# psipred/DMPfold2

Measured on AMD Instinct MI355X. Metric: structures/s at L=300, N_seq=2000, 10 iters+100 min, higher is better.
Workload: dtype f32 with full-width operands on the bf16 matrix cores (option precision = 2): convolution operands split exactly into 3 bf16 pieces (24 significand bits), the 6 piece products above 2^-24 accumulated in f32 by v_mfma_f32_32x32x16_bf16; vertical GRU the same way (3 bf16 pieces per operand, 6 products

## Files before the change

dmpfold2_amd/csrc/vgru.h:

```cpp
#pragma once
#include "common.h"

namespace dmp {

typedef float f32x16 __attribute__((ext_vector_type(16)));
typedef _Float16 vg_f16x8 __attribute__((ext_vector_type(8)));

struct VStatic {
  const uint4* wx[2];
  const uint4* wh[2];
  const float* bias[2];
  float inv_scale[2];
  float* hT[2][2];
  uint16_t* hH[2][2];
};
constexpr int VG_TB = 32;


__host__ __device__ inline int vgru_pitch(int L) { return (L + VG_TB - 1) / VG_TB * VG_TB; }

typedef unsigned vg_u32x4 __attribute__((ext_vector_type(4)));

constexpr int VG_MAX_MEMBERS = 8;

struct VMember { const uint8_t* msa; int N, L, tile0, pad; };
struct VGroupRec { int t0, t_end, nmem, pad; VMember mem[VG_MAX_MEMBERS]; };
static_assert(sizeof(VGroupRec) <= 256, "dmp_ctx_create sizes vgru_run for 256 bytes");

typedef float vp_f32x4 __attribute__((ext_vector_type(4)));
constexpr int VP_WL0_SLOTS = 4 * 4 * 6 * 64;
constexpr int VP_RED_SLOTS = 4 * 14 * 64;
constexpr int VP_TAB_FLOATS = 3 * 24 * 16;
constexpr int VP_LDS_BYTES = (VP_WL0_SLOTS + VP_RED_SLOTS) * 16 + VP_TAB_FLOATS * 4;
constexpr int VP_MAX_XCD_TILES = 64;
constexpr int VP_GRID = 256;
struct VPSync { unsigned count[8]; unsigned pad[24]; unsigned flag[8][32]; };
static_assert(sizeof(VPSync) == 128 + 1024, "VPSync layout");
constexpr unsigned VP_BARRIER_SPINS = 800000u;
constexpr unsigned VP_BARRIER_SPINS_FIRST = 8u * VP_BARRIER_SPINS;

__device__ __forceinline__ bool vp_claim_slice(VPSync* __restrict__ sync, int* __restrict__ fault, int barrier, int tid,
                                               int* sh_u, int* sh_abort, unsigned& xcc, int& u) {
  if (barrier) {
    asm volatile("s_getreg_b32 %0, hwreg(HW_REG_XCC_ID)" : "=s"(xcc));
    xcc &= 7u;
    if (tid == 0) {
      *sh_u = (int)__hip_atomic_fetch_add(&sync->count[xcc], 1u, __ATOMIC_RELAXED, __HIP_MEMORY_SCOPE_AGENT);
      *sh_abort = 0;
    }
  } else {
    xcc = blockIdx.x & 7u;
    if (tid == 0) { *sh_u = (int)(blockIdx.x >> 3); *sh_abort = 0; }
  }
  __syncthreads();
  u = *sh_u;
  if (u >= 32) {
    if (tid == 0) atomicOr(fault, DMP_FAULT_VGRU_HANDOFF);
    return false;
  }
  return true;
}

__device__ __forceinline__ bool vp_tile_table(const VGroupRec* __restrict__ rec, int nmem, int c_lo, int c_hi, int tid,
                                              int* __restrict__ fault, int (*sh_tile)[4], unsigned long long* sh_msa) {
  if (c_hi - c_lo > VP_MAX_XCD_TILES) {
    if (tid == 0) atomicOr(fault, DMP_FAULT_VGRU_HANDOFF);
    return false;
  }
  for (int i = tid; i < c_hi - c_lo; i += 256) {
    const int tile = c_lo + i;
    int mi = 0;
    for (int m = 1; m < VG_MAX_MEMBERS; ++m)
      if (m < nmem && tile >= rec->mem[m].tile0) mi = m;
    sh_tile[i][0] = rec->mem[mi].N;
    sh_tile[i][1] = rec->mem[mi].L;
    sh_tile[i][2] = (tile - rec->mem[mi].tile0) * VG_TB;
    sh_tile[i][3] = mi;
  }
  if (tid < VG_MAX_MEMBERS) sh_msa[tid] = tid < nmem ? (unsigned long long)rec->mem[tid].msa : 0ull;
  __syncthreads();
  return true;
}

__device__ __forceinline__ int vp_next_active(const int (*sh_tile)[4], int c_lo, int c_hi, int ct, int t) {
  for (; ct < c_hi; ++ct) {
    const int N = __builtin_amdgcn_readfirstlane(sh_tile[ct - c_lo][0]);
    if (t < N || (t >= 1 && t <= N)) break;
  }
  return ct;
}

__device__ __forceinline__ void vp_store_partials(vp_f32x4* red, int w, int lane, const vp_f32x4 (&a0)[3][2],
                                                  const vp_f32x4 (&a1)[4][2]) {
#pragma unroll
  for (int g = 0; g < 3; ++g)
#pragma unroll
    for (int nt = 0; nt < 2; ++nt) red[(w * 14 + g * 2 + nt) * 64 + lane] = a0[g][nt];
#pragma unroll
  for (int g = 0; g < 4; ++g)
#pragma unroll
    for (int nt = 0; nt < 2; ++nt) red[(w * 14 + 6 + g * 2 + nt) * 64 + lane] = a1[g][nt];
}

__device__ __forceinline__ vp_f32x4 vp_quarter_sum(const vp_f32x4* red, int a, int flane) {
  return ((red[(0 * 14 + a) * 64 + flane] + red[(1 * 14 + a) * 64 + flane]) + red[(2 * 14 + a) * 64 + flane]) +
         red[(3 * 14 + a) * 64 + flane];
}

__device__ __forceinline__ vp_f32x4 vp_onehot_term(const float* tab, int g, int code, int fg) {
  const float* t = tab + (g * 24 + code) * 16 + 4 * fg;
  return vp_f32x4{t[0], t[1], t[2], t[3]};
}

__device__ __forceinline__ float vp_gru_cell(float s_r, float s_z, float s_hn, float s_in, float b_r, float b_z, float b_in,
                                             float b_hn, float h) {
  const float rg = 1.0f / (1.0f + expf(-(s_r + b_r)));
  const float zg = 1.0f / (1.0f + expf(-(s_z + b_z)));
  const float ng = tanhf((s_in + b_in) + rg * (s_hn + b_hn));
  return (h - ng) * zg + ng;
}

__device__ __forceinline__ bool vp_row_barrier(VPSync* __restrict__ sync, int* __restrict__ fault, unsigned xcc, int u, int w,
                                               int lane, int tid, int t, int t_lo, int* sh_abort) {
  asm volatile("s_waitcnt vmcnt(0)" ::: "memory");
  __syncthreads();
  const unsigned epoch = (unsigned)(t - t_lo + 1);
  if (tid == 0) asm volatile("global_store_dword %0, %1, off" :: "v"(&sync->flag[xcc][u]), "v"(epoch) : "memory");
  if (w == 0) {
    const unsigned* fp = &sync->flag[xcc][lane & 31];
    bool ok = false;
    const unsigned bound = t == t_lo ? VP_BARRIER_SPINS_FIRST : VP_BARRIER_SPINS;
    for (unsigned spins = 0; spins < bound && !ok; ++spins) {
      unsigned v;
      asm volatile("global_load_dword %0, %1, off sc1\n\ts_waitcnt vmcnt(0)" : "=v"(v) : "v"(fp) : "memory");
      ok = __builtin_amdgcn_ballot_w64(v < epoch) == 0ull;
    }
    if (!ok && lane == 0) { atomicOr(fault, DMP_FAULT_VGRU_HANDOFF); *sh_abort = 1; }
  }
  __syncthreads();
  return *sh_abort != 0;
}


struct VStaticF32 {
  const float4* wh0;
  const float4* wx1;
  const float4* wh1;
  const float* wx0;
  const float* bias[2];
  float* hT[2][2];
  uint4* wq;
};
typedef void (*vgru_f32_kernel_t)(VStaticF32, const VGroupRec*, VPSync*, int*, int, int, int, int);

inline int vgru_f32_launch(vgru_f32_kernel_t kernel, dmp_ctx* lead, int t_lo, int t_hi, hipStream_t s) {
  const int nt = lead->vg_ntiles;
  if (t_hi > lead->vg_maxN + 1) t_hi = lead->vg_maxN + 1;
  if (t_lo < 0) t_lo = 0;
  if (t_lo >= t_hi) return DMP_OK;
  const Weights& W = lead->W;
  VStaticF32 st{};
  st.wh0 = reinterpret_cast<const float4*>(W.v_f32[0]);
  st.wx1 = reinterpret_cast<const float4*>(W.v_f32[1]);
  st.wh1 = reinterpret_cast<const float4*>(W.v_f32[2]);
  st.wx0 = W.v_wx0f;
  st.bias[0] = W.v_b0; st.bias[1] = W.v_b1;
  for (int l = 0; l < 2; ++l)
    for (int p = 0; p < 2; ++p) st.hT[l][p] = lead->hT[l][p];
  st.wq = reinterpret_cast<uint4*>(lead->vgru_wq);
  const VGroupRec* rec = reinterpret_cast<const VGroupRec*>(lead->vgru_run);
  VPSync* sync = reinterpret_cast<VPSync*>(lead->vgru_sync);
  if (lead->vgru_persist && lead->vgru_persist_ok) {
    CoResident guard(lead, s, true);
    if (guard.status()) return guard.status();
    DMP_HIP(hipMemsetAsync(sync, 0, sizeof(VPSync), s));
    hipLaunchKernelGGL(kernel, dim3(VP_GRID - (lead->vgru_debug_drop_wg ? 1 : 0)), dim3(256), VP_LDS_BYTES, s, st, rec, sync,
                       lead->seq_abort, t_lo, t_hi, nt, 1);
    DMP_LAUNCH_CHECK();
    return guard.done();
  }
  for (int t = t_lo; t < t_hi; ++t)
    hipLaunchKernelGGL(kernel, dim3(VP_GRID), dim3(256), VP_LDS_BYTES, s, st, rec, sync, lead->seq_abort, t, t + 1, nt, 0);
  DMP_LAUNCH_CHECK();
  return DMP_OK;
}

int vgru_f32_group_steps(dmp_ctx* lead, int t_lo, int t_hi, hipStream_t s);
int vgru_f32_kernel_attrs(dmp_ctx* c);
int vgru_x3_group_steps(dmp_ctx* lead, int t_lo, int t_hi, hipStream_t s);
int vgru_x3_kernel_attrs(dmp_ctx* c);

}
```

dmpfold2_amd/csrc/vgru_x3.hip:

```cpp
#include "vgru.h"

namespace dmp {

typedef __bf16 vx_bf16x8 __attribute__((ext_vector_type(8)));

__device__ __forceinline__ void vx_split8(const float (&w)[8], vx_bf16x8 (&p)[3]) {
  float r[8];
#pragma unroll
  for (int e = 0; e < 8; ++e) { const __bf16 h = (__bf16)w[e]; p[0][e] = h; r[e] = w[e] - (float)h; }
#pragma unroll
  for (int e = 0; e < 8; ++e) { const __bf16 h = (__bf16)r[e]; p[1][e] = h; r[e] = r[e] - (float)h; }
#pragma unroll
  for (int e = 0; e < 8; ++e) p[2][e] = (__bf16)r[e];
}

__device__ __forceinline__ vp_f32x4 vx_mfma(vx_bf16x8 a, vx_bf16x8 b, vp_f32x4 c) {
  return __builtin_amdgcn_mfma_f32_16x16x32_bf16(a, b, c, 0, 0, 0);
}

__device__ __forceinline__ float vx_sigmoid(float x) { return 1.0f / (1.0f + expf(-x)); }

constexpr int VX_KS = 4;
constexpr int VX_WQ = 6;
constexpr size_t VX_WQ_BYTES = (size_t)VP_GRID * 4 * VX_KS * VX_WQ * 64 * 16;
static_assert(4 * VX_KS * 3 * 2 * 64 == VP_WL0_SLOTS, "two pieces of layer 0's weights fill the LDS area of the f16 form's pieces");

constexpr int VX_SC1 = 16;

struct VxAddr {
  __amdgpu_buffer_rsrc_t r0, r1, rq;
  unsigned vlane, vq;
  unsigned k4w, krot, Lb;
};

__device__ __forceinline__ void vx_request(vp_f32x4 (&F)[4][2], int u4, unsigned S, unsigned col, const VxAddr& A) {
  const unsigned base = ((A.k4w + 8 * ((S + A.krot) & (VX_KS - 1))) * A.Lb + col + (u4 & 1) * 16) * 16;
#pragma unroll
  for (int h = 0; h < 2; ++h)
    F[u4][h] = __builtin_bit_cast(vp_f32x4, __builtin_amdgcn_raw_buffer_load_b128(u4 < 2 ? A.r1 : A.r0, A.vlane, base + h * A.Lb * 16, VX_SC1));
}

__device__ __forceinline__ void vx_split_octet(const vp_f32x4 (&f)[2], vx_bf16x8 (&q)[3]) {
  const float wv[8] = {f[0][0], f[0][1], f[0][2], f[0][3], f[1][0], f[1][1], f[1][2], f[1][3]};
  vx_split8(wv, q);
}

template <bool ACT0, bool ACT1>
__device__ __forceinline__ void vx_tile_products(vp_f32x4 (&a0)[3][2], vp_f32x4 (&a1)[4][2], const vx_bf16x8 (&PA)[VX_KS][3][3],
                                                 const vx_bf16x8 (&PB)[VX_KS][3][2], vx_bf16x8 (&WB)[3], vx_bf16x8 (&WC)[3],
                                                 const vx_bf16x8* __restrict__ wl0w, vp_f32x4 (&F)[4][2], vx_bf16x8 (&Q)[2][3],
                                                 const VxAddr& A, unsigned tcol, unsigned ncol) {
#pragma unroll
  for (int S = 0; S < VX_KS; ++S) {
    vx_bf16x8 T[3][2];
#pragma unroll
    for (int g = 0; g < 3; ++g) {
      T[g][0] = wl0w[((S * 3 + g) * 2 + 0) * 64];
      T[g][1] = wl0w[((S * 3 + g) * 2 + 1) * 64];
    }
    __builtin_amdgcn_sched_barrier(0);
#pragma unroll
    for (int u4 = 0; u4 < 4; ++u4) {
      const int unit = 4 * S + u4, nt = u4 & 1, cur = unit & 1, nxt = cur ^ 1, n4 = (u4 + 1) & 3;
      vx_bf16x8 (&P)[3] = Q[cur];
      const int nm = u4 < 2 ? (ACT1 ? 18 : 0) : (ACT0 ? 18 : 0) + (ACT1 ? 18 : 0);
#pragma unroll
      for (int pb = 2; pb >= 0; --pb)
#pragma unroll
        for (int pa = 2 - pb; pa >= 0; --pa)
#pragma unroll
          for (int g = 0; g < 3; ++g) {
            if (u4 < 2) {
              if (ACT1) a1[g][nt] = vx_mfma(pa == 2 ? WB[g] : PB[S][g][pa == 2 ? 0 : pa], P[pb], a1[g][nt]);
            } else {
              if (ACT0) a0[g][nt] = vx_mfma(pa == 2 ? WC[g] : T[g][pa == 2 ? 0 : pa], P[pb], a0[g][nt]);
              if (ACT1) a1[g == 2 ? 3 : g][nt] = vx_mfma(PA[S][g][pa], P[pb], a1[g == 2 ? 3 : g][nt]);
            }
          }
      vx_split_octet(F[n4], Q[nxt]);
      vx_request(F, n4, (unit + 5) >> 2 & (VX_KS - 1), unit + 5 < 4 * VX_KS ? tcol : ncol, A);
      if (u4 == 1) {
#pragma unroll
        for (int g = 0; g < 3; ++g)
          WB[g] = __builtin_bit_cast(vx_bf16x8, __builtin_amdgcn_raw_buffer_load_b128(A.rq, A.vq, (((S + 1) & (VX_KS - 1)) * VX_WQ + g) * 1024, 0));
      }
      if (u4 == 3) {
#pragma unroll
        for (int g = 0; g < 3; ++g)
          WC[g] = __builtin_bit_cast(vx_bf16x8, __builtin_amdgcn_raw_buffer_load_b128(A.rq, A.vq, (((S + 1) & (VX_KS - 1)) * VX_WQ + 3 + g) * 1024, 0));
      }
#pragma unroll
      for (int i = 0; i < 36; ++i)
        if (i < nm) {
          __builtin_amdgcn_sched_group_barrier(0x008, 1, 0);
          __builtin_amdgcn_sched_group_barrier(0x002, 3, 0);
        }
      __builtin_amdgcn_sched_barrier(0);
    }
  }
}

__global__ __launch_bounds__(256) __attribute__((amdgpu_waves_per_eu(1, 1)))
void vgru_persist_x3_kernel(VStaticF32 st, const VGroupRec* __restrict__ rec, VPSync* __restrict__ sync,
                            int* __restrict__ fault, int t_lo, int t_hi, int ntiles, int barrier) {
  extern __shared__ __attribute__((aligned(16))) unsigned char vx_smem[];
  vx_bf16x8* wl0 = reinterpret_cast<vx_bf16x8*>(vx_smem);
  vp_f32x4* red = reinterpret_cast<vp_f32x4*>(vx_smem + VP_WL0_SLOTS * 16);
  float* tab = reinterpret_cast<float*>(vx_smem + (VP_WL0_SLOTS + VP_RED_SLOTS) * 16);
  __shared__ int sh_u, sh_abort;
  __shared__ __attribute__((aligned(16))) float sh_bias[2][4][16];
  __shared__ int sh_tile[VP_MAX_XCD_TILES][5];
  __shared__ unsigned long long sh_msa[VG_MAX_MEMBERS];
  const int tid = threadIdx.x, lane = tid & 63;
  const int w = __builtin_amdgcn_readfirstlane(tid >> 6);
  unsigned xcc;
  if (barrier) {
    asm volatile("s_getreg_b32 %0, hwreg(HW_REG_XCC_ID)" : "=s"(xcc));
    xcc &= 7u;
    if (tid == 0) {
      sh_u = (int)__hip_atomic_fetch_add(&sync->count[xcc], 1u, __ATOMIC_RELAXED, __HIP_MEMORY_SCOPE_AGENT);
      sh_abort = 0;
    }
  } else {
    xcc = blockIdx.x & 7u;
    if (tid == 0) { sh_u = (int)(blockIdx.x >> 3); sh_abort = 0; }
  }
  __syncthreads();
  const int u = sh_u;
  if (u >= 32) {
    if (tid == 0) atomicOr(fault, DMP_FAULT_VGRU_HANDOFF);
    return;
  }
  const int j0 = 16 * u, lr = lane & 15, lq = lane >> 4;
  const int Lb = ntiles * VG_TB;
  const int c_lo = (int)(((long long)ntiles * xcc) / 8), c_hi = (int)(((long long)ntiles * (xcc + 1)) / 8);

  vx_bf16x8 PA[VX_KS][3][3], PB[VX_KS][3][2];
  uint4* wqw = st.wq + (size_t)(blockIdx.x * 4 + w) * VX_KS * VX_WQ * 64 + lane;
#pragma unroll
  for (int S = 0; S < VX_KS; ++S)
#pragma unroll
    for (int g = 0; g < 3; ++g) {
      float wa[8], wb[8], wc[8];
#pragma unroll
      for (int h = 0; h < 2; ++h) {
        const int64_t off = (int64_t)(g * 128 + 32 * w + 8 * ((S + u) & (VX_KS - 1)) + 2 * lq + h) * 512 + j0 + lr;
        const float4 a = st.wx1[off], b = st.wh1[off], c = st.wh0[off];
        wa[4 * h + 0] = a.x; wa[4 * h + 1] = a.y; wa[4 * h + 2] = a.z; wa[4 * h + 3] = a.w;
        wb[4 * h + 0] = b.x; wb[4 * h + 1] = b.y; wb[4 * h + 2] = b.z; wb[4 * h + 3] = b.w;
        wc[4 * h + 0] = c.x; wc[4 * h + 1] = c.y; wc[4 * h + 2] = c.z; wc[4 * h + 3] = c.w;
      }
      vx_split8(wa, PA[S][g]);
      vx_bf16x8 pb[3], pc[3];
      vx_split8(wb, pb);
      vx_split8(wc, pc);
      PB[S][g][0] = pb[0];
      PB[S][g][1] = pb[1];
      wl0[(((w * VX_KS + S) * 3 + g) * 2 + 0) * 64 + lane] = pc[0];
      wl0[(((w * VX_KS + S) * 3 + g) * 2 + 1) * 64 + lane] = pc[1];
      wqw[(S * VX_WQ + g) * 64] = __builtin_bit_cast(uint4, pb[2]);
      wqw[(S * VX_WQ + 3 + g) * 64] = __builtin_bit_cast(uint4, pc[2]);
    }
  asm volatile("s_waitcnt vmcnt(0)" ::: "memory");
  const vx_bf16x8* wl0w = wl0 + w * VX_KS * 3 * 2 * 64 + lane;
  if (tid < 128) sh_bias[tid >> 6][(tid >> 4) & 3][tid & 15] = st.bias[tid >> 6][((tid >> 4) & 3) * 512 + j0 + (tid & 15)];
  for (int i = tid; i < 3 * 22 * 16; i += 256) {
    const int g = i / (22 * 16), code = (i / 16) % 22, row = i & 15;
    tab[(g * 24 + code) * 16 + row] = st.wx0[(g * 22 + code) * 512 + j0 + row];
  }
  const int fl = __builtin_amdgcn_readfirstlane(tid >> 7), fg = (tid >> 5) & 3, fc = tid & 31;
  const int flane = 16 * fg + (fc & 15), fnt = fc >> 4;
  const int j4 = j0 + 4 * fg;
  const int nmem = rec->nmem;
  if (c_hi - c_lo > VP_MAX_XCD_TILES) {
    if (tid == 0) atomicOr(fault, DMP_FAULT_VGRU_HANDOFF);
    return;
  }
  for (int i = tid; i < c_hi - c_lo; i += 256) {
    const int tile = c_lo + (i + u) % (c_hi - c_lo);
    int mi = 0;
    for (int m = 1; m < VG_MAX_MEMBERS; ++m)
      if (m < nmem && tile >= rec->mem[m].tile0) mi = m;
    sh_tile[i][0] = rec->mem[mi].N;
    sh_tile[i][1] = rec->mem[mi].L;
    sh_tile[i][2] = (tile - rec->mem[mi].tile0) * VG_TB;
    sh_tile[i][3] = mi;
    sh_tile[i][4] = tile;
  }
  if (tid < VG_MAX_MEMBERS) sh_msa[tid] = tid < nmem ? (unsigned long long)rec->mem[tid].msa : 0ull;
  __syncthreads();
  auto next_active = [&](int ct, int t) {
    for (; ct < c_hi; ++ct) {
      const int N = __builtin_amdgcn_readfirstlane(sh_tile[ct - c_lo][0]);
      if (t < N || (t >= 1 && t <= N)) break;
    }
    return ct;
  };
  const unsigned state_bytes = (unsigned)(128 * Lb * 16);

  VxAddr A;
  A.k4w = (unsigned)(32 * w);
  A.krot = (unsigned)(u & (VX_KS - 1));
  A.Lb = (unsigned)Lb;
  A.vlane = (unsigned)((2 * lq * Lb + lr) * 16);
  A.vq = (unsigned)(lane * 16);
  A.rq = __builtin_amdgcn_make_buffer_rsrc(st.wq + (size_t)(blockIdx.x * 4 + w) * VX_KS * VX_WQ * 64, 0, VX_KS * VX_WQ * 1024, 0x00020000);
  vx_bf16x8 WB[3], WC[3];
#pragma unroll
  for (int g = 0; g < 3; ++g) {
    WB[g] = __builtin_bit_cast(vx_bf16x8, __builtin_amdgcn_raw_buffer_load_b128(A.rq, A.vq, g * 1024, 0));
    WC[g] = __builtin_bit_cast(vx_bf16x8, __builtin_amdgcn_raw_buffer_load_b128(A.rq, A.vq, (3 + g) * 1024, 0));
  }
  for (int t = t_lo; t < t_hi; ++t) {
    const int par = t & 1;
    A.r0 = __builtin_amdgcn_make_buffer_rsrc(st.hT[0][par], 0, state_bytes, 0x00020000);
    A.r1 = __builtin_amdgcn_make_buffer_rsrc(st.hT[1][par ^ 1], 0, state_bytes, 0x00020000);
    const __amdgpu_buffer_rsrc_t rh = fl ? A.r1 : A.r0;
    float* hnext = fl ? st.hT[1][par] : st.hT[0][par ^ 1];
    int ct = next_active(c_lo, t);
    vp_f32x4 F[4][2];
    vx_bf16x8 Q[2][3];
    if (ct < c_hi) {
      const unsigned col0 = (unsigned)(__builtin_amdgcn_readfirstlane(sh_tile[ct - c_lo][4]) * VG_TB);
#pragma unroll
      for (int u4 = 0; u4 < 4; ++u4) vx_request(F, u4, 0, col0, A);
      vx_split_octet(F[0], Q[0]);
      vx_request(F, 0, 1, col0, A);
    }
    while (ct < c_hi) {
      const int nx = next_active(ct + 1, t);
      const int ncol = __builtin_amdgcn_readfirstlane(sh_tile[(nx < c_hi ? nx : ct) - c_lo][4]) * VG_TB;
      const int N = __builtin_amdgcn_readfirstlane(sh_tile[ct - c_lo][0]);
      const int L = __builtin_amdgcn_readfirstlane(sh_tile[ct - c_lo][1]);
      const bool act0 = t < N, act1 = t >= 1 && t <= N;
      const int tcol = __builtin_amdgcn_readfirstlane(sh_tile[ct - c_lo][4]) * VG_TB;
      vp_f32x4 a0[3][2], a1[4][2];
#pragma unroll
      for (int g = 0; g < 3; ++g) { a0[g][0] = vp_f32x4{0, 0, 0, 0}; a0[g][1] = vp_f32x4{0, 0, 0, 0}; }
#pragma unroll
      for (int g = 0; g < 4; ++g) { a1[g][0] = vp_f32x4{0, 0, 0, 0}; a1[g][1] = vp_f32x4{0, 0, 0, 0}; }
      if (act0 && act1)
        vx_tile_products<true, true>(a0, a1, PA, PB, WB, WC, wl0w, F, Q, A, (unsigned)tcol, (unsigned)ncol);
      else if (act0)
        vx_tile_products<true, false>(a0, a1, PA, PB, WB, WC, wl0w, F, Q, A, (unsigned)tcol, (unsigned)ncol);
      else
        vx_tile_products<false, true>(a0, a1, PA, PB, WB, WC, wl0w, F, Q, A, (unsigned)tcol, (unsigned)ncol);
      const int b = tcol + fc;
      const int64_t hoff = ((int64_t)(j4 >> 2) * Lb + b) * 4;
      float hp[4];
#pragma unroll
      for (int i = 0; i < 4; ++i)
        hp[i] = __builtin_bit_cast(float, __builtin_amdgcn_raw_buffer_load_b32(rh, (unsigned)(hoff * 4 + 4 * i), 0, VX_SC1));
      const int bm = sh_tile[ct - c_lo][2] + fc;
      const uint8_t* msa = reinterpret_cast<const uint8_t*>(sh_msa[sh_tile[ct - c_lo][3]]);
      const int code = (fl == 0 && act0 && bm < L) ? (int)msa[(int64_t)t * L + bm] : 0;
#pragma unroll
      for (int g = 0; g < 3; ++g)
#pragma unroll
        for (int nt = 0; nt < 2; ++nt) red[(w * 14 + g * 2 + nt) * 64 + lane] = a0[g][nt];
#pragma unroll
      for (int g = 0; g < 4; ++g)
#pragma unroll
        for (int nt = 0; nt < 2; ++nt) red[(w * 14 + 6 + g * 2 + nt) * 64 + lane] = a1[g][nt];
      __syncthreads();
      if (fl ? act1 : act0) {
        const int nq = fl ? 4 : 3, base = fl ? 6 : 0;
        vp_f32x4 sum[4];
#pragma unroll
        for (int q = 0; q < 4; ++q) {
          if (q < nq) {
            const int a = base + q * 2 + fnt;
            sum[q] = ((red[(0 * 14 + a) * 64 + flane] + red[(1 * 14 + a) * 64 + flane]) + red[(2 * 14 + a) * 64 + flane]) +
                     red[(3 * 14 + a) * 64 + flane];
          }
        }
        if (fl == 0) {
          const float* tr = tab + (0 * 24 + code) * 16 + 4 * fg;
          const float* tz = tab + (1 * 24 + code) * 16 + 4 * fg;
          const float* tn = tab + (2 * 24 + code) * 16 + 4 * fg;
#pragma unroll
          for (int i = 0; i < 4; ++i) { sum[0][i] += tr[i]; sum[1][i] += tz[i]; sum[3][i] = tn[i]; }
        }
        const float* br = &sh_bias[fl][0][4 * fg];
        const float* bz = &sh_bias[fl][1][4 * fg];
        const float* bi = &sh_bias[fl][2][4 * fg];
        const float* bh = &sh_bias[fl][3][4 * fg];
        float hn[4];
#pragma unroll
        for (int i = 0; i < 4; ++i) {
          const float rg = vx_sigmoid(sum[0][i] + br[i]);
          const float zg = vx_sigmoid(sum[1][i] + bz[i]);
          const float ng = tanhf((sum[3][i] + bi[i]) + rg * (sum[2][i] + bh[i]));
          hn[i] = (hp[i] - ng) * zg + ng;
        }
        *reinterpret_cast<float4*>(hnext + hoff) = make_float4(hn[0], hn[1], hn[2], hn[3]);
      }
      __syncthreads();
      ct = nx;
    }
    if (!barrier) break;
    if (vp_row_barrier(sync, fault, xcc, u, w, lane, tid, t, t_lo, &sh_abort)) break;
  }
}

size_t vgru_x3_stream_bytes() { return VX_WQ_BYTES; }

int vgru_x3_kernel_attrs(dmp_ctx* c) {
  (void)c;
  DMP_HIP(hipFuncSetAttribute((const void*)vgru_persist_x3_kernel, hipFuncAttributeMaxDynamicSharedMemorySize, VP_LDS_BYTES));
  return DMP_OK;
}

int vgru_x3_group_steps(dmp_ctx* lead, int t_lo, int t_hi, hipStream_t s) {
  return vgru_f32_launch(vgru_persist_x3_kernel, lead, t_lo, t_hi, s);
}

}
```

Measured before the change: 4.372.

## Keep small bf16 weight pieces resident in LDS by staging the reduction

```diff
diff --git a/dmpfold2_amd/csrc/vgru.h b/dmpfold2_amd/csrc/vgru.h
--- a/dmpfold2_amd/csrc/vgru.h
+++ b/dmpfold2_amd/csrc/vgru.h
@@ -32,6 +32,9 @@
 constexpr int VP_RED_SLOTS = 4 * 14 * 64;
 constexpr int VP_TAB_FLOATS = 3 * 24 * 16;
 constexpr int VP_LDS_BYTES = (VP_WL0_SLOTS + VP_RED_SLOTS) * 16 + VP_TAB_FLOATS * 4;
+constexpr int VX_STAGE_ACCS = 4;
+constexpr int VX_STAGE_SLOTS = 4 * VX_STAGE_ACCS * 64;
+constexpr int VX_RES_SLOTS = (VP_RED_SLOTS - VX_STAGE_SLOTS) / (4 * 64);
 constexpr int VP_MAX_XCD_TILES = 64;
 constexpr int VP_GRID = 256;
 struct VPSync { unsigned count[8]; unsigned pad[24]; unsigned flag[8][32]; };
diff --git a/dmpfold2_amd/csrc/vgru_x3.hip b/dmpfold2_amd/csrc/vgru_x3.hip
--- a/dmpfold2_amd/csrc/vgru_x3.hip
+++ b/dmpfold2_amd/csrc/vgru_x3.hip
@@ -45,11 +45,22 @@
   vx_split8(wv, q);
 }
 
+__device__ __forceinline__ constexpr int vx_res_slot(int S, int kind, int g) {
+  return (S * 2 + kind) * 3 + g < VX_RES_SLOTS ? (S * 2 + kind) * 3 + g : -1;
+}
+
+__device__ __forceinline__ vx_bf16x8 vx_small_piece(int S, int kind, int g, const vx_bf16x8* __restrict__ wres, const VxAddr& A) {
+  const int slot = vx_res_slot(S, kind, g);
+  if (slot >= 0) return wres[slot * 64];
+  return __builtin_bit_cast(vx_bf16x8, __builtin_amdgcn_raw_buffer_load_b128(A.rq, A.vq, (S * VX_WQ + 3 * kind + g) * 1024, 0));
+}
+
 template <bool ACT0, bool ACT1>
 __device__ __forceinline__ void vx_tile_products(vp_f32x4 (&a0)[3][2], vp_f32x4 (&a1)[4][2], const vx_bf16x8 (&PA)[VX_KS][3][3],
                                                  const vx_bf16x8 (&PB)[VX_KS][3][2], vx_bf16x8 (&WB)[3], vx_bf16x8 (&WC)[3],
-                                                 const vx_bf16x8* __restrict__ wl0w, vp_f32x4 (&F)[4][2], vx_bf16x8 (&Q)[2][3],
-                                                 const VxAddr& A, unsigned tcol, unsigned ncol) {
+                                                 const vx_bf16x8* __restrict__ wl0w, const vx_bf16x8* __restrict__ wres,
+                                                 vp_f32x4 (&F)[4][2], vx_bf16x8 (&Q)[2][3], const VxAddr& A, unsigned tcol,
+                                                 unsigned ncol) {
 #pragma unroll
   for (int S = 0; S < VX_KS; ++S) {
     vx_bf16x8 T[3][2];
@@ -81,13 +92,11 @@
       vx_request(F, n4, (unit + 5) >> 2 & (VX_KS - 1), unit + 5 < 4 * VX_KS ? tcol : ncol, A);
       if (u4 == 1) {
 #pragma unroll
-        for (int g = 0; g < 3; ++g)
-          WB[g] = __builtin_bit_cast(vx_bf16x8, __builtin_amdgcn_raw_buffer_load_b128(A.rq, A.vq, (((S + 1) & (VX_KS - 1)) * VX_WQ + g) * 1024, 0));
+        for (int g = 0; g < 3; ++g) WB[g] = vx_small_piece((S + 1) & (VX_KS - 1), 0, g, wres, A);
       }
       if (u4 == 3) {
 #pragma unroll
-        for (int g = 0; g < 3; ++g)
-          WC[g] = __builtin_bit_cast(vx_bf16x8, __builtin_amdgcn_raw_buffer_load_b128(A.rq, A.vq, (((S + 1) & (VX_KS - 1)) * VX_WQ + 3 + g) * 1024, 0));
+        for (int g = 0; g < 3; ++g) WC[g] = vx_small_piece((S + 1) & (VX_KS - 1), 1, g, wres, A);
       }
 #pragma unroll
       for (int i = 0; i < 36; ++i)
@@ -106,6 +115,7 @@
   extern __shared__ __attribute__((aligned(16))) unsigned char vx_smem[];
   vx_bf16x8* wl0 = reinterpret_cast<vx_bf16x8*>(vx_smem);
   vp_f32x4* red = reinterpret_cast<vp_f32x4*>(vx_smem + VP_WL0_SLOTS * 16);
+  vx_bf16x8* res = reinterpret_cast<vx_bf16x8*>(vx_smem + (VP_WL0_SLOTS + VX_STAGE_SLOTS) * 16);
   float* tab = reinterpret_cast<float*>(vx_smem + (VP_WL0_SLOTS + VP_RED_SLOTS) * 16);
   __shared__ int sh_u, sh_abort;
   __shared__ __attribute__((aligned(16))) float sh_bias[2][4][16];
@@ -158,11 +168,14 @@
       PB[S][g][1] = pb[1];
       wl0[(((w * VX_KS + S) * 3 + g) * 2 + 0) * 64 + lane] = pc[0];
       wl0[(((w * VX_KS + S) * 3 + g) * 2 + 1) * 64 + lane] = pc[1];
-      wqw[(S * VX_WQ + g) * 64] = __builtin_bit_cast(uint4, pb[2]);
-      wqw[(S * VX_WQ + 3 + g) * 64] = __builtin_bit_cast(uint4, pc[2]);
+      if (vx_res_slot(S, 0, g) >= 0) res[(w * VX_RES_SLOTS + vx_res_slot(S, 0, g)) * 64 + lane] = pb[2];
+      else wqw[(S * VX_WQ + g) * 64] = __builtin_bit_cast(uint4, pb[2]);
+      if (vx_res_slot(S, 1, g) >= 0) res[(w * VX_RES_SLOTS + vx_res_slot(S, 1, g)) * 64 + lane] = pc[2];
+      else wqw[(S * VX_WQ + 3 + g) * 64] = __builtin_bit_cast(uint4, pc[2]);
     }
   asm volatile("s_waitcnt vmcnt(0)" ::: "memory");
   const vx_bf16x8* wl0w = wl0 + w * VX_KS * 3 * 2 * 64 + lane;
+  const vx_bf16x8* wres = res + w * VX_RES_SLOTS * 64 + lane;
   if (tid < 128) sh_bias[tid >> 6][(tid >> 4) & 3][tid & 15] = st.bias[tid >> 6][((tid >> 4) & 3) * 512 + j0 + (tid & 15)];
   for (int i = tid; i < 3 * 22 * 16; i += 256) {
     const int g = i / (22 * 16), code = (i / 16) % 22, row = i & 15;
@@ -208,8 +221,8 @@
   vx_bf16x8 WB[3], WC[3];
 #pragma unroll
   for (int g = 0; g < 3; ++g) {
-    WB[g] = __builtin_bit_cast(vx_bf16x8, __builtin_amdgcn_raw_buffer_load_b128(A.rq, A.vq, g * 1024, 0));
-    WC[g] = __builtin_bit_cast(vx_bf16x8, __builtin_amdgcn_raw_buffer_load_b128(A.rq, A.vq, (3 + g) * 1024, 0));
+    WB[g] = vx_small_piece(0, 0, g, wres, A);
+    WC[g] = vx_small_piece(0, 1, g, wres, A);
   }
   for (int t = t_lo; t < t_hi; ++t) {
     const int par = t & 1;
@@ -240,11 +253,11 @@
 #pragma unroll
       for (int g = 0; g < 4; ++g) { a1[g][0] = vp_f32x4{0, 0, 0, 0}; a1[g][1] = vp_f32x4{0, 0, 0, 0}; }
       if (act0 && act1)
-        vx_tile_products<true, true>(a0, a1, PA, PB, WB, WC, wl0w, F, Q, A, (unsigned)tcol, (unsigned)ncol);
+        vx_tile_products<true, true>(a0, a1, PA, PB, WB, WC, wl0w, wres, F, Q, A, (unsigned)tcol, (unsigned)ncol);
       else if (act0)
-        vx_tile_products<true, false>(a0, a1, PA, PB, WB, WC, wl0w, F, Q, A, (unsigned)tcol, (unsigned)ncol);
+        vx_tile_products<true, false>(a0, a1, PA, PB, WB, WC, wl0w, wres, F, Q, A, (unsigned)tcol, (unsigned)ncol);
       else
-        vx_tile_products<false, true>(a0, a1, PA, PB, WB, WC, wl0w, F, Q, A, (unsigned)tcol, (unsigned)ncol);
+        vx_tile_products<false, true>(a0, a1, PA, PB, WB, WC, wl0w, wres, F, Q, A, (unsigned)tcol, (unsigned)ncol);
       const int b = tcol + fc;
       const int64_t hoff = ((int64_t)(j4 >> 2) * Lb + b) * 4;
       float hp[4];
@@ -254,26 +267,24 @@
       const int bm = sh_tile[ct - c_lo][2] + fc;
       const uint8_t* msa = reinterpret_cast<const uint8_t*>(sh_msa[sh_tile[ct - c_lo][3]]);
       const int code = (fl == 0 && act0 && bm < L) ? (int)msa[(int64_t)t * L + bm] : 0;
-#pragma unroll
-      for (int g = 0; g < 3; ++g)
-#pragma unroll
-        for (int nt = 0; nt < 2; ++nt) red[(w * 14 + g * 2 + nt) * 64 + lane] = a0[g][nt];
-#pragma unroll
-      for (int g = 0; g < 4; ++g)
-#pragma unroll
-        for (int nt = 0; nt < 2; ++nt) red[(w * 14 + 6 + g * 2 + nt) * 64 + lane] = a1[g][nt];
-      __syncthreads();
-      if (fl ? act1 : act0) {
-        const int nq = fl ? 4 : 3, base = fl ? 6 : 0;
-        vp_f32x4 sum[4];
-#pragma unroll
-        for (int q = 0; q < 4; ++q) {
-          if (q < nq) {
-            const int a = base + q * 2 + fnt;
-            sum[q] = ((red[(0 * 14 + a) * 64 + flane] + red[(1 * 14 + a) * 64 + flane]) + red[(2 * 14 + a) * 64 + flane]) +
-                     red[(3 * 14 + a) * 64 + flane];
-          }
-        }
+      const bool fin = fl ? act1 : act0;
+      vp_f32x4 sum[4];
+#pragma unroll
+      for (int q = 0; q < 4; ++q) {
+        if (q) __syncthreads();
+#pragma unroll
+        for (int nt = 0; nt < 2; ++nt) {
+          if (q < 3) red[(w * VX_STAGE_ACCS + nt) * 64 + lane] = a0[q][nt];
+          red[(w * VX_STAGE_ACCS + 2 + nt) * 64 + lane] = a1[q][nt];
+        }
+        __syncthreads();
+        if (fin && (fl || q < 3)) {
+          const int a = 2 * fl + fnt;
+          sum[q] = ((red[(0 * VX_STAGE_ACCS + a) * 64 + flane] + red[(1 * VX_STAGE_ACCS + a) * 64 + flane]) +
+                    red[(2 * VX_STAGE_ACCS + a) * 64 + flane]) + red[(3 * VX_STAGE_ACCS + a) * 64 + flane];
+        }
+      }
+      if (fin) {
         if (fl == 0) {
           const float* tr = tab + (0 * 24 + code) * 16 + 4 * fg;
           const float* tz = tab + (1 * 24 + code) * 16 + 4 * fg;
```

New measurement: 4.412, median of 6. Within noise of the previous version (+0.9%).
